# Chlumsky/msdfgen

Measured on AMD Instinct MI355X. Metric: MSDF glyphs/sec (64x64, fp32), higher is better.
Workload: dtype f64

## Files before the change

### msdfgen_amd/csrc/msdf_device.hpp

```cpp
#pragma once

#include <stdint.h>
#include <stddef.h>
#include <math.h>
#include <float.h>

#if defined(__HIPCC__)
#define MSDF_HD __host__ __device__ inline
#define MSDF_NOINLINE __attribute__((noinline))
#define MSDF_NOUNROLL _Pragma("clang loop unroll(disable)")
#define MSDF_UNROLL _Pragma("unroll")
#if defined(__HIP_DEVICE_COMPILE__)
#define MSDF_UNIFORM(x) __builtin_amdgcn_readfirstlane(x)
#else
#define MSDF_UNIFORM(x) (x)
#endif
#else
#define MSDF_HD inline
#define MSDF_NOINLINE
#define MSDF_NOUNROLL
#define MSDF_UNROLL
#define MSDF_UNIFORM(x) (x)
#endif

// ... 107 lines not shown
MSDF_HD V2 EdgeRec::EP0() const { return ld(ep0); }
MSDF_HD V2 EdgeRec::EP1() const { return ld(ep1); }

MSDF_HD V2 normalize(V2 a, bool allowZero) {
    double len = vlen(a);
    if (len != 0)
        return mk(a.x/len, a.y/len);
    return mk(0, allowZero ? 0. : 1.);
}

MSDF_HD V2 normalizeLen(V2 a, double len, bool allowZero) {
    if (len != 0)
        return mk(a.x/len, a.y/len);
    return mk(0, allowZero ? 0. : 1.);
}

MSDF_HD V2 orthonormalFalse(V2 a) {
    double len = vlen(a);
    if (len != 0)
        return mk(a.y/len, -a.x/len);
    return mk(0, -1.);
}

MSDF_HD V2 mixv(V2 a, V2 b, double w) { return (1.-w)*a+w*b; }
MSDF_HD double nonZeroSign(double n) { return n > 0 ? 1. : -1.; }
MSDF_HD double dmin(double a, double b) { return b < a ? b : a; }
MSDF_HD double dmax(double a, double b) { return a < b ? b : a; }
MSDF_HD double cmax(double a, double b) { return __builtin_fmax(a, b); }
MSDF_HD double cmin(double a, double b) { return __builtin_fmin(a, b); }
MSDF_HD double median(double a, double b, double c) { return dmax(dmin(a, b), dmin(dmax(a, b), c)); }
MSDF_HD float fmin_(float a, float b) { return b < a ? b : a; }
MSDF_HD float fmax_(float a, float b) { return a < b ? b : a; }
MSDF_HD float medianf(float a, float b, float c) { return fmax_(fmin_(a, b), fmin_(fmax_(a, b), c)); }
MSDF_HD float mixf(float a, float b, double w) { return (float) ((1.-w)*a+w*b); }

MSDF_HD double divExact(double a, double b, double y) {
    const double q = a*y;
    const double r = fma(-b, q, a);
    return fma(r, y, q);
}

MSDF_HD bool divSafe(double b) {
    const double m = fabs(b);
    if (!(m > 1e-100 && m < 1e100))
        return false;
    int e;
    const double f = frexp(m, &e);
    return f != 1-0x1p-53;
}


MSDF_HD int solveQuadratic(double x[2], double a, double b, double c) {
    if (a == 0 || fabs(b) > 1e12*fabs(a)) {
        if (b == 0) {
            if (c == 0)
                return -1;
            return 0;
        }
        x[0] = -c/b;
        return 1;
    }
    double dscr = b*b-4*a*c;
    if (dscr > 0) {
        dscr = msdfSqrt(dscr);
        x[0] = (-b+dscr)/(2*a);
        x[1] = (-b-dscr)/(2*a);
// ... 890 lines not shown
```

### msdfgen_amd/csrc/msdf_ec.hpp

```cpp
#pragma once

#include "msdf_device.hpp"

namespace msdfhip {

enum { EC_ERROR = 1, EC_PROTECTED = 2 };
enum { EC_MODE_DISABLED = 0, EC_MODE_INDISCRIMINATE = 1, EC_MODE_EDGE_PRIORITY = 2, EC_MODE_EDGE_ONLY = 3 };
enum { EC_DO_NOT_CHECK = 0, EC_CHECK_AT_EDGE = 1, EC_ALWAYS_CHECK = 2 };

#define MSDF_ARTIFACT_T_EPSILON .01
#define MSDF_PROTECTION_RADIUS_TOLERANCE 1.001

struct SdfView {
    const float *px;
    int w, h, N;
    int flip;
    MSDF_HD const float *native(int x, int y) const { return px+((size_t) y*w+x)*N; }
    MSDF_HD const float *shape(int x, int y) const { return native(x, flip ? h-1-y : y); }
};

struct EcParams {
    Xform t;
    double minDeviationRatio, minImproveRatio;
    float radiusH, radiusV, radiusD;
// ... 104 lines not shown
    l = clampi(l, sdf.w-1), r = clampi(r, sdf.w-1);
    b = clampi(b, sdf.h-1), t = clampi(t, sdf.h-1);
    const float *lb = sdf.shape(l, b), *rb = sdf.shape(r, b), *lt = sdf.shape(l, t), *rt = sdf.shape(r, t);
    for (int i = 0; i < 3; ++i)
        out[i] = mixf(mixf(lb[i], rb[i], lr), mixf(lt[i], rt[i], lr), bt);
}

template <class Query>
MSDF_HD bool evaluate(const Classifier<Query> &c, double t, float m, int flags) {
    (void) m;
    if (!c.shapeAware)
        return (flags&2) != 0;
    if (flags&1) {
        if (flags&2)
            return true;
        V2 tVector = t*c.direction;
        float oldMSD[3], newMSD[3];
        V2 sdfCoord = c.sdfCoord+tVector;
        interpolate3(oldMSD, *c.sdf, sdfCoord);
        double aWeight = (1-fabs(tVector.x))*(1-fabs(tVector.y));
        float aPSD = medianf(c.msd[0], c.msd[1], c.msd[2]);
        newMSD[0] = (float) (oldMSD[0]+aWeight*(aPSD-c.msd[0]));
        newMSD[1] = (float) (oldMSD[1]+aWeight*(aPSD-c.msd[1]));
        newMSD[2] = (float) (oldMSD[2]+aWeight*(aPSD-c.msd[2]));
        float oldPSD = medianf(oldMSD[0], oldMSD[1], oldMSD[2]);
        float newPSD = medianf(newMSD[0], newMSD[1], newMSD[2]);
        V2 q = c.shapeCoord+mk(tVector.x*c.p->texelX, tVector.y*c.p->texelY);
        float refPSD = mapDistance(c.p->t, (*c.query)(q));
        return c.p->minImproveRatio*fabsf(newPSD-refPSD) < (double) fabsf(oldPSD-refPSD);
    }
    return false;
}

MSDF_HD float interpolatedMedianLin(const float *a, const float *b, double t) {
    return medianf(mixf(a[0], b[0], t), mixf(a[1], b[1], t), mixf(a[2], b[2], t));
}

MSDF_HD float interpolatedMedianQuad(const float *a, const float *l, const float *q, double t) {
    return (float) median(t*(t*q[0]+l[0])+a[0], t*(t*q[1]+l[1])+a[1], t*(t*q[2]+l[2])+a[2]);
}

template <class Query>
MSDF_HD bool hasLinearArtifactInner(const Classifier<Query> &cl, float am, float bm, const float *a, const float *b, float dA, float dB) {
    double t = (double) dA/(dA-dB);
    if (t > MSDF_ARTIFACT_T_EPSILON && t < 1-MSDF_ARTIFACT_T_EPSILON) {
        float xm = interpolatedMedianLin(a, b, t);
        return evaluate(cl, t, xm, rangeTest(cl, 0, 1, t, am, bm, xm));
    }
    return false;
}

template <class Query>
MSDF_HD bool hasDiagonalArtifactInner(const Classifier<Query> &cl, float am, float dm, const float *a, const float *l, const float *q,
                                      float dA, float dBC, float dD, double tEx0, double tEx1) {
    double t[2];
    int solutions = solveQuadratic(t, dD-dBC+dA, dBC-dA-dA, dA);
    for (int i = 0; i < solutions; ++i) {
        if (t[i] > MSDF_ARTIFACT_T_EPSILON && t[i] < 1-MSDF_ARTIFACT_T_EPSILON) {
            float xm = interpolatedMedianQuad(a, l, q, t[i]);
            int rangeFlags = rangeTest(cl, 0, 1, t[i], am, dm, xm);
            if (tEx0 > 0 && tEx0 < 1) {
                double tEnd0 = 0, tEnd1 = 1;
                float em0 = am, em1 = dm;
                float ex = interpolatedMedianQuad(a, l, q, tEx0);
                if (tEx0 > t[i])
                    tEnd1 = tEx0, em1 = ex;
                else
                    tEnd0 = tEx0, em0 = ex;
                rangeFlags |= rangeTest(cl, tEnd0, tEnd1, t[i], em0, em1, xm);
            }
            if (tEx1 > 0 && tEx1 < 1) {
// ... 134 lines not shown
```

### msdfgen_amd/csrc/msdf_ec_fast.hpp

```cpp
#pragma once

#include "msdf_ec.hpp"

namespace msdfhip {

enum { EC_DEFER = 0x80 };

enum { EC_V_ERROR = 1,
       EC_V_CHECK = 2,
       EC_V_COND = 4,
       EC_V_HELD = 8 };
enum { EC_ORDER_EAGER = 0, EC_ORDER_LAZY = 1, EC_ORDER_LAZY_HELD = 2 };

MSDF_HD bool ecHasBasePass(const EcParams &p) { return p.distanceCheck == EC_DO_NOT_CHECK || (p.distanceCheck == EC_CHECK_AT_EDGE && p.mode != EC_MODE_EDGE_ONLY); }
MSDF_HD bool ecHasShapePass(const EcParams &p) { return p.distanceCheck == EC_ALWAYS_CHECK || p.distanceCheck == EC_CHECK_AT_EDGE; }
MSDF_HD bool ecLazyProtect(const EcParams &p) { return p.mode == EC_MODE_EDGE_PRIORITY && p.distanceCheck == EC_CHECK_AT_EDGE; }

struct FastCtx {
    double span;
    bool p1;
    bool pShape;
    bool basePass, shapePass;
    int order;
};

MSDF_HD int rangeTest2(const FastCtx &c, double at, double bt, double xt, float am, float bm, float xm) {
    const bool inversion = (am > .5f && bm > .5f && xm <= .5f) || (am < .5f && bm < .5f && xm >= .5f);
    const bool outside = medianf(am, bm, xm) != xm;
    const bool candBase = c.basePass && (inversion || (!c.p1 && outside));
    const bool candShape = c.shapePass && (inversion || (!c.pShape && outside));
    const bool candCond = c.order != EC_ORDER_EAGER && !inversion && outside;
    if (!(candBase || candShape || candCond))
        return 0;
    const double axSpan = (xt-at)*c.span, bxSpan = (bt-xt)*c.span;
    const int f = (xm >= am-axSpan && xm <= am+axSpan && xm >= bm-bxSpan && xm <= bm+bxSpan) ? 1 : 3;
    return (candBase ? f : 0)|(candShape ? f<<2 : 0)|(candCond && f == 3 ? 16 : 0);
}

MSDF_HD int judge(int flags) {
    const int cond = (flags&16) ? EC_V_COND : 0;
    if (flags&2)
        return EC_V_ERROR|cond;
    const int fs = (flags>>2)&3;
    if (fs&1)
        return ((fs&2) ? EC_V_ERROR : EC_V_CHECK)|cond;
    return cond;
}

MSDF_HD bool quadraticMayHaveRootInRange(double a, double b, double c) {
    if (a == 0 || fabs(b) > 1e12*fabs(a))
        return true;
    const double lo = .005, hi = .995;
    const double mag = fabs(a)+fabs(b)+fabs(c);
    const double eps = 1e-9*mag;
    const double flo = (a*lo+b)*lo+c, fhi = (a*hi+b)*hi+c;
    if (!(flo > eps && fhi > eps) && !(flo < -eps && fhi < -eps))
        return true;
    const double s = flo > 0 ? 1. : -1.;
    const double as = a*s, bs = b*s, cs = c*s;
    if (as <= 0)
        return false;
    if (!(-bs > 2*as*lo*(1-1e-9) && -bs < 2*as*hi*(1+1e-9)))
        return false;
    return !(4*as*cs-bs*bs > 1e-9*mag*mag);
}

MSDF_HD bool bernsteinMayHaveRoot(float dA, float dBC, float dD) {
    const float m = fmaxf(fmaxf(fabsf(dA), fabsf(dBC)), fabsf(dD));
    const float eps = 1e-5f*m;
    const float h = .5f*dBC;
    return !((dA > eps && h > eps && dD > eps) || (dA < -eps && h < -eps && dD < -eps));
}

MSDF_HD bool edgeBetweenTexelsChannelFast(const float *a, const float *b, int channel) {
    const double n = a[channel]-.5;
    const double d = a[channel]-b[channel];
    if (!((n > 0 && d > 0 && n < d) || (n < 0 && d < 0 && n > d)))
        return false;
    const double t = n/d;
    if (t > 0 && t < 1) {
        float c[3] = { mixf(a[0], b[0], t), mixf(a[1], b[1], t), mixf(a[2], b[2], t) };
        return medianf(c[0], c[1], c[2]) == c[channel];
    }
    return false;
}

MSDF_HD int edgeBetweenTexelsFast(const float *a, const float *b) {
    return 1*(int) edgeBetweenTexelsChannelFast(a, b, 0)+2*(int) edgeBetweenTexelsChannelFast(a, b, 1)+4*(int) edgeBetweenTexelsChannelFast(a, b, 2);
}

struct DiagonalRoots {
    double r0, r1;
    double ex0, ex1;
    int m, ne;
};

MSDF_HD bool diagonalRootsInRange(DiagonalRoots &d, double qa, double qb, double qc, float l0, float q0, float l1, float q1) {
    d.m = 0, d.ne = 0;
    d.r0 = d.r1 = d.ex0 = d.ex1 = 0;
    if (!quadraticMayHaveRootInRange(qa, qb, qc))
        return false;
    double t[2] = { 0, 0 };
    const int solutions = solveQuadratic(t, qa, qb, qc);
    const bool in0 = (solutions > 0)&(t[0] > MSDF_ARTIFACT_T_EPSILON)&(t[0] < 1-MSDF_ARTIFACT_T_EPSILON);
    const bool in1 = (solutions > 1)&(t[1] > MSDF_ARTIFACT_T_EPSILON)&(t[1] < 1-MSDF_ARTIFACT_T_EPSILON);
    d.m = (int) in0+(int) in1;
    if (!d.m)
        return false;
    d.r0 = in0 ? t[0] : t[1], d.r1 = t[1];
    const double tEx0 = -.5*l0/q0, tEx1 = -.5*l1/q1;
    const bool e0 = (tEx0 > 0)&(tEx0 < 1), e1 = (tEx1 > 0)&(tEx1 < 1);
    d.ne = (int) e0+(int) e1;
    d.ex0 = e0 ? tEx0 : tEx1, d.ex1 = tEx1;
    return true;
}

MSDF_HD int diagonalUnitFlags(const FastCtx &cx, float am, float dm, const float *a, const float *l, const float *q, double t, double tEx, bool extremum, float xm) {
    if (!extremum)
        return rangeTest2(cx, 0, 1, t, am, dm, xm);
    double tEnd0 = 0, tEnd1 = 1;
    float em0 = am, em1 = dm;
    const float ex = interpolatedMedianQuad(a, l, q, tEx);
    if (tEx > t)
        tEnd1 = tEx, em1 = ex;
    else
        tEnd0 = tEx, em0 = ex;
    return rangeTest2(cx, tEnd0, tEnd1, t, em0, em1, xm);
}

template <class Sink>
MSDF_HD bool diagonalRootVerdict(const FastCtx &cx, int rangeFlags, double t, int &verdict, Sink &sink) {
    const int v = judge(rangeFlags);
    verdict |= v;
    if (v&EC_V_CHECK) {
        const bool held = (verdict&EC_V_COND) != 0;
        if (held)
            verdict |= EC_V_HELD;
        if (held == (cx.order == EC_ORDER_LAZY_HELD))
            sink(t);
    }
    return (verdict&EC_V_ERROR) != 0;
}

template <class Sink>
MSDF_HD int diagonalPairFast(const FastCtx &cx, float am, float dm, const float *a, const float *l, const float *q,
                             float dA, float dBC, float dD, float l0, float q0, float l1, float q1, Sink &sink) {
    const double qa = dD-dBC+dA, qb = dBC-dA-dA, qc = dA;
    DiagonalRoots d;
    if (!diagonalRootsInRange(d, qa, qb, qc, l0, q0, l1, q1))
        return 0;
    int verdict = 0;
    MSDF_UNROLL
    for (int i = 0; i < 2; ++i) {
        if (i >= d.m)
            break;
        const double t = i ? d.r1 : d.r0;
        const float xm = interpolatedMedianQuad(a, l, q, t);
        int rangeFlags = diagonalUnitFlags(cx, am, dm, a, l, q, t, 0, false, xm);
        if (d.ne > 0)
            rangeFlags |= diagonalUnitFlags(cx, am, dm, a, l, q, t, d.ex0, true, xm);
        if (d.ne > 1)
            rangeFlags |= diagonalUnitFlags(cx, am, dm, a, l, q, t, d.ex1, true, xm);
        if (diagonalRootVerdict(cx, rangeFlags, t, verdict, sink))
            return verdict;
    }
    return verdict;
}

struct Neighbourhood {
    float v[3][3][3];
    float dev[3][3];
    unsigned cls[3][3];
    unsigned valid;
};

MSDF_HD float ecTexelDeviation(const float *t) { return fabsf(medianf(t[0], t[1], t[2])-.5f); }

enum { EC_CLS_INSIDE = 0x8000 };
MSDF_HD unsigned ecTexelClassWord(const float *t) {
    unsigned w = EC_CLS_INSIDE;
    MSDF_UNROLL
    for (int j = 0; j < 3; ++j) {
        const float d = t[j == 2 ? 0 : j+1]-t[j];
        w |= (d > 0 ? 1u<<j : 0u)|(d < 0 ? 8u<<j : 0u)|(d == 0 ? 64u<<j : 0u);
    }
    return w;
}

MSDF_HD unsigned ecValidFromWords(const Neighbourhood &nb) {
    unsigned valid = 0;
    MSDF_UNROLL
    for (int m = 0; m < 9; ++m)
        valid |= (nb.cls[m/3][m%3]&EC_CLS_INSIDE) ? 1u<<m : 0u;
    return valid;
}

MSDF_HD void loadNeighbourhood(Neighbourhood &nb, const SdfView &sdf, int x, int yn) {
    MSDF_UNROLL
    for (int dy = -1; dy <= 1; ++dy) {
        MSDF_UNROLL
        for (int dx = -1; dx <= 1; ++dx) {
            const int nx = x+dx, ny = yn+dy;
            const bool in = nx >= 0 && ny >= 0 && nx < sdf.w && ny < sdf.h;
            const float *t = sdf.native(in ? nx : x, in ? ny : yn);
            nb.v[dy+1][dx+1][0] = t[0], nb.v[dy+1][dx+1][1] = t[1], nb.v[dy+1][dx+1][2] = t[2];
            nb.dev[dy+1][dx+1] = ecTexelDeviation(t);
            nb.cls[dy+1][dx+1] = in ? ecTexelClassWord(t) : 0u;
        }
    }
    nb.valid = ecValidFromWords(nb);
}

template <class Emit>
MSDF_HD void texelProtectPairs(const Neighbourhood &nb, const EcParams &p, Emit &emit) {
    const float sdev = nb.dev[1][1];
    MSDF_UNROLL
    for (int dy = -1; dy <= 1; ++dy) {
        MSDF_UNROLL
        for (int dx = -1; dx <= 1; ++dx) {
            if (!dx && !dy)
                continue;
            if (!(nb.cls[dy+1][dx+1]&EC_CLS_INSIDE))
                continue;
            const float radius = dy == 0 ? p.radiusH : dx == 0 ? p.radiusV : p.radiusD;
            const float odev = nb.dev[dy+1][dx+1];
            const bool selfIsA = dy > 0 || (dy == 0 && dx > 0);
            const float sum = selfIsA ? sdev+odev : odev+sdev;
            if (sum < radius)
                emit((dy+1)*3+(dx+1));
        }
    }
}

MSDF_HD bool evaluateProtectPair(const float *self, const float *other, int m, bool swapRows = false) {
    const int dy = m/3-1, dx = m%3-1;
    const bool selfIsA = (swapRows ? dy < 0 : dy > 0) || (dy == 0 && dx > 0);
    const int mask = selfIsA ? edgeBetweenTexelsFast(self, other) : edgeBetweenTexelsFast(other, self);
    return extremeChannelInMask(self, medianf(self[0], self[1], self[2]), mask);
}

MSDF_HD bool protectedByEdgesNb(const Neighbourhood &nb, const EcParams &p, int flip = 0) {
    struct Items {
        unsigned char m[8];
        int n;
        MSDF_HD void operator()(int mm) { m[n++] = (unsigned char) mm; }
    } items;
    items.n = 0;
    texelProtectPairs(nb, p, items);
    for (int i = 0; i < items.n; ++i)
        if (evaluateProtectPair(nb.v[1][1], nb.v[items.m[i]/3][items.m[i]%3], items.m[i], p.shapeRows && flip))
            return true;
    return false;
}

MSDF_HD int ecNeighbourDx(int k) { return k < 4 ? (k == 0 ? -1 : k == 2 ? 1 : 0) : ((k&1) ? 1 : -1); }
MSDF_HD int ecNeighbourDy(int k) { return k < 4 ? (k == 1 ? -1 : k == 3 ? 1 : 0) : ((k&2) ? 1 : -1); }

template <class Emit>
MSDF_HD void texelCandidatePairs(const Neighbourhood &nb, Emit &emit) {
    const float *c = nb.v[1][1];
    const float cdev = nb.dev[1][1];
    const unsigned cw = nb.cls[1][1];
    MSDF_UNROLL
    for (int k = 0; k < 4; ++k) {
        const int dx = k == 0 ? -1 : k == 2 ? 1 : 0, dy = k == 1 ? -1 : k == 3 ? 1 : 0;
        const unsigned nw = nb.cls[dy+1][dx+1];
        const unsigned opposite = ((cw&(nw>>3))|((cw>>3)&nw))&7u;
        const unsigned m = cdev >= nb.dev[dy+1][dx+1] ? opposite : 0u;
        if (m) {
            if (m&1u)
                emit(k, 0);
            if (m&2u)
                emit(k, 1);
            if (m&4u)
                emit(k, 2);
        }
    }
    MSDF_UNROLL
    for (int k = 4; k < 8; ++k) {
        const int dx = (k&1) ? 1 : -1, dy = (k&2) ? 1 : -1;
        const unsigned dw = nb.cls[dy+1][dx+1];
        if (!(((dw&EC_CLS_INSIDE) != 0)&(cdev >= nb.dev[dy+1][dx+1])))
            continue;
        const float *d = nb.v[dy+1][dx+1];
        const float *b = nb.v[1][dx+1], *cc = nb.v[dy+1][1];
        const unsigned zeroAD = cw&dw;
        MSDF_UNROLL
        for (int j = 0; j < 3; ++j) {
            const int i0 = j, i1 = j == 2 ? 0 : j+1;
            const float dA = c[i1]-c[i0], dBC = b[i1]-b[i0]+cc[i1]-cc[i0], dD = d[i1]-d[i0];
            if ((zeroAD&(64u<<j)) && dBC == 0)
                continue;
            if (bernsteinMayHaveRoot(dA, dBC, dD))
                emit(k, j);
        }
    }
}

MSDF_HD float pick3(const float *v, int i) { return i == 0 ? v[0] : i == 1 ? v[1] : v[2]; }

template <class Sink>
MSDF_HD int evaluatePair(const float *c, const float *n, const float *hb, const float *vc, const EcParams &p, bool p1, int flip, int k, int j, Sink &sink,
                         int order = EC_ORDER_EAGER) {
    FastCtx cx;
    cx.basePass = ecHasBasePass(p);
    cx.shapePass = ecHasShapePass(p);
    cx.order = order;
    cx.p1 = order != EC_ORDER_EAGER || p1;
    cx.pShape = (p.distanceCheck == EC_CHECK_AT_EDGE) ? true : cx.p1;
    const int dx = ecNeighbourDx(k), dy = ecNeighbourDy(k);
    const int i0 = j, i1 = j == 2 ? 0 : j+1;
    const float cm = medianf(c[0], c[1], c[2]), nm = medianf(n[0], n[1], n[2]);
    if (k < 4) {
        if (order == EC_ORDER_LAZY_HELD)
            return 0;
        cx.span = dy == 0 ? p.hSpan : p.vSpan;
        const float dA = pick3(c, i1)-pick3(c, i0), dB = pick3(n, i1)-pick3(n, i0);
        const double t = (double) dA/(dA-dB);
        if (t > MSDF_ARTIFACT_T_EPSILON && t < 1-MSDF_ARTIFACT_T_EPSILON) {
            const float xm = interpolatedMedianLin(c, n, t);
            const int v = judge(rangeTest2(cx, 0, 1, t, cm, nm, xm));
            if (v&EC_V_CHECK)
                sink(t, dx, flip ? -dy : dy);
            return v;
        }
        return 0;
    }
    cx.span = p.dSpan;
    const float *a = c, *b = hb, *cc = vc, *d = n;
    const float abc[3] = { a[0]-b[0]-cc[0], a[1]-b[1]-cc[1], a[2]-b[2]-cc[2] };
    const float l[3] = { -a[0]-abc[0], -a[1]-abc[1], -a[2]-abc[2] };
    const float q[3] = { d[0]+abc[0], d[1]+abc[1], d[2]+abc[2] };
    const float a3[3] = { a[0], a[1], a[2] };
    struct DirSink {
        Sink &sink;
        int dx, dy;
        MSDF_HD void operator()(double t) { sink(t, dx, dy); }
    } dirSink = { sink, dx, flip ? -dy : dy };
    const float dA = pick3(a, i1)-pick3(a, i0), dBC = pick3(b, i1)-pick3(b, i0)+pick3(cc, i1)-pick3(cc, i0), dD = pick3(d, i1)-pick3(d, i0);
    return diagonalPairFast(cx, cm, nm, a3, l, q, dA, dBC, dD, pick3(l, i0), pick3(q, i0), pick3(l, i1), pick3(q, i1), dirSink);
}

template <class Sink>
MSDF_HD int texelFindFast(const Neighbourhood &nb, const EcParams &p, bool p1, int flip, Sink &sink, int order = EC_ORDER_EAGER) {
    struct Items {
        unsigned char k[24], j[24];
        int n;
        MSDF_HD void operator()(int kk, int jj) { k[n] = (unsigned char) kk, j[n] = (unsigned char) jj; ++n; }
    } items;
    items.n = 0;
    texelCandidatePairs(nb, items);
    int verdict = 0;
    for (int i = 0; i < items.n; ++i) {
        const int k = items.k[i], dx = ecNeighbourDx(k), dy = ecNeighbourDy(k);
        verdict |= evaluatePair(nb.v[1][1], nb.v[dy+1][dx+1], nb.v[1][dx+1], nb.v[dy+1][1], p, p1, flip, k, items.j[i], sink, order);
    }
    return verdict;
}

MSDF_HD bool protectedByCornerList(const int *corners, int nCorners, int x, int ys) {
    for (int i = 0; i < nCorners; ++i) {
        const int l = corners[2*i], b = corners[2*i+1];
        if ((x == l || x == l+1) && (ys == b || ys == b+1))
            return true;
    }
    return false;
}

MSDF_HD bool ecNeedsProtection(int verdict) { return ((verdict&EC_V_COND) && !(verdict&EC_V_ERROR)) || (verdict&EC_V_HELD); }

template <class Sink>
MSDF_HD int ecTexelFast(const SdfView &sdf, const EcParams &p, const int *corners, int nCorners, int x, int yn, Sink &sink, bool allowLazy = true) {
    const int ys = sdf.flip ? sdf.h-1-yn : yn;
    Neighbourhood nb;
    loadNeighbourhood(nb, sdf, x, yn);
    int st = 0, verdict;
    if (allowLazy && ecLazyProtect(p)) {
        verdict = texelFindFast(nb, p, true, sdf.flip, sink, EC_ORDER_LAZY);
        if (ecNeedsProtection(verdict)) {
            if (!(protectedByCornerList(corners, nCorners, x, ys) || protectedByEdgesNb(nb, p, sdf.flip)))
                verdict |= EC_V_ERROR;
            else if (verdict&EC_V_HELD)
                texelFindFast(nb, p, true, sdf.flip, sink, EC_ORDER_LAZY_HELD);
        }
    } else {
        if (p.mode == EC_MODE_EDGE_PRIORITY) {
            if (protectedByCornerList(corners, nCorners, x, ys) || protectedByEdgesNb(nb, p, sdf.flip))
                st |= EC_PROTECTED;
// ... 33 lines not shown
```

### msdfgen_amd/csrc/msdf_kernels.hpp

```cpp
#pragma once

#include <hip/hip_runtime.h>
#include "msdf_device.hpp"
#include "msdf_prep.hpp"
#include "msdf_ec.hpp"
#include "msdf_ec_fast.hpp"
#include "msdf_cull.hpp"
#include "msdf_scanline.hpp"
#include "msdf_shapeprep.hpp"
#include "msdf_frame.hpp"
#include "msdf_legacy.hpp"
#include "../../include/msdfgen_hip.h"

namespace msdfhip {

#ifndef MSDF_DISTANCE_WAVES_PER_SIMD
#define MSDF_DISTANCE_WAVES_PER_SIMD 4
#endif
constexpr int TILE = 8;
constexpr int WAVE = 64;
constexpr int REC_DOUBLES = sizeof(EdgeRec)/sizeof(double);

struct BatchView {
    int nGlyphs;
// ... 1013 lines not shown

#ifndef MSDF_EC_FAST_WAVES_PER_SIMD
#define MSDF_EC_FAST_WAVES_PER_SIMD 7
#endif
enum { EC_HALO = TILE+2, EC_QUEUE_CAP = WAVE*24, EC_PROTECT_QUEUE_CAP = WAVE*8 };
__host__ __device__ inline size_t ecFastLdsBytes(int maxEdges, int n) {
    return (size_t) EC_HALO*EC_HALO*n*sizeof(float)+(WAVE+4)*sizeof(int)
           +(EC_QUEUE_CAP+EC_PROTECT_QUEUE_CAP)*sizeof(unsigned short);
}

__device__ __forceinline__ bool ecTileCornerTexel(const int *list, int nCorners, int tx, int ty, int height, int flip, int lane) {
    const int lxT = lane&(TILE-1), lyT = lane>>3;
    const int xT = tx*TILE+lxT, ysT = flip ? height-1-(ty*TILE+lyT) : ty*TILE+lyT;
    const int x0 = tx*TILE, x1 = tx*TILE+TILE-1;
    const int ya = flip ? height-1-(ty*TILE+TILE-1) : ty*TILE, yb = flip ? height-1-ty*TILE : ty*TILE+TILE-1;
    bool cornerTexel = false;
    for (int base = 0; base < nCorners; base += WAVE) {
        const int k = base+lane;
        int l = 0, b = 0;
        bool near = false;
        if (k < nCorners) {
            l = list[2*k], b = list[2*k+1];
            near = l+1 >= x0 && l <= x1 && b+1 >= ya && b <= yb;
        }
        for (unsigned long long mask = __ballot(near); mask; mask &= mask-1) {
            const int src = __ffsll((long long) mask)-1;
            const int cl = __builtin_amdgcn_readlane(l, src), cb = __builtin_amdgcn_readlane(b, src);
            cornerTexel = cornerTexel || ((xT == cl || xT == cl+1) && (ysT == cb || ysT == cb+1));
        }
    }
    return cornerTexel;
}

template <int N>
__device__ __forceinline__ void ecRunProtectQueue(const float *halo, const unsigned short *protectQueue, int nProtect, int *verdictLds, int lane, bool swapRows = false) {
    for (int base = 0; base < nProtect; base += WAVE) {
        const int it = base+lane;
        if (it >= nProtect)
            continue;
        const unsigned item = protectQueue[it];
        const int s = item&63, m = item>>6;
        const int sx = s&(TILE-1), sy = s>>3;
        const float *self = halo+((sy+1)*EC_HALO+sx+1)*N, *other = halo+((sy+m/3)*EC_HALO+sx+m%3)*N;
        if (evaluateProtectPair(self, other, m, swapRows))
            atomicOr(&verdictLds[s], 0x100);
    }
}

struct EcPushProtect {
    unsigned short *queue;
    int *count;
    int lane;
    __device__ void operator()(int m) { queue[atomicAdd(count, 1)] = (unsigned short) (lane|m<<6); }
};

template <int N, int ORDER = -1, bool SIZED = false, bool SHAPE_ROWS = false>
__device__ __forceinline__ void ecFastBody(const BatchView &batch, const MsdfHipGlyph *glyphs, int width, int height, int tilesX, int tilesPerGlyph,
          const float *src, float *out, uint8_t *stencilOut, const MsdfHipConfig &cfg, const EcGlyphParams *glyphParams, EcCandidate *cands, unsigned seg,
          int maxEdges, const int *corners, const unsigned blockId, int *smemFast, const int sinkSlots = 0, const int sinkSlot = 0, const int32_t *__restrict__ dims = NULL) {
    const GlyphWork wk = decodeItem(blockId, batch.nGlyphs, tilesPerGlyph);
    if (!wk.valid)
        return;
    const int boxW = SIZED ? MSDF_UNIFORM(dims[2*wk.g]) : width, boxH = SIZED ? MSDF_UNIFORM(dims[2*wk.g+1]) : height;
    if (SIZED && ((wk.tile%tilesX)*TILE >= boxW || (wk.tile/tilesX)*TILE >= boxH))
        return;
    float *halo = reinterpret_cast<float *>(smemFast);
    int *verdictLds = reinterpret_cast<int *>(halo+EC_HALO*EC_HALO*N);
    int *itemCount = verdictLds+WAVE;
    unsigned short *queue = reinterpret_cast<unsigned short *>(itemCount+4);
    unsigned short *protectQueue = queue+EC_QUEUE_CAP;
    struct TexelClass {
        float dev;
        unsigned cls;
    };
    TexelClass *classLds = reinterpret_cast<TexelClass *>(queue+EC_QUEUE_CAP)-EC_HALO*EC_HALO;
    static_assert((EC_QUEUE_CAP*sizeof(unsigned short))%sizeof(TexelClass) == 0 && EC_QUEUE_CAP*sizeof(unsigned short) >= EC_HALO*EC_HALO*sizeof(TexelClass)
                  && 2*WAVE >= EC_HALO*EC_HALO && WAVE%EC_HALO == 4 && WAVE/EC_HALO == 6, "classLds overlays the queue's tail; the halo is staged in two rounds");
    const int lane = threadIdx.x;
    const MsdfHipGlyph gd = glyphs[wk.g];
    EcParams p;
    p.t = loadXform(gd);
    p.minDeviationRatio = cfg.min_deviation_ratio;
    p.minImproveRatio = cfg.min_improve_ratio;
    p.mode = cfg.ec_mode, p.distanceCheck = cfg.ec_distance_check, p.overlap = cfg.overlap_support, p.stageLimit = 0;
    const EcGlyphParams gp = glyphParams[wk.g];
    p.hSpan = gp.hSpan, p.vSpan = gp.vSpan, p.dSpan = gp.dSpan, p.texelX = gp.texelX, p.texelY = gp.texelY;
    p.radiusH = gp.radiusH, p.radiusV = gp.radiusV, p.radiusD = gp.radiusD;
    const int tx = wk.tile%tilesX, ty = wk.tile/tilesX;

    const bool lazy = ORDER < 0 ? ecLazyProtect(p) : ORDER != 0;
    bool cornerTexel = false;
    if (p.mode == EC_MODE_EDGE_PRIORITY && !lazy)
        cornerTexel = ecTileCornerTexel(corners+2*(size_t) gp.cornerBegin, gp.nCorners, tx, ty, boxH, gd.flip, lane);

    const ptrdiff_t rowStep = (ptrdiff_t) boxW*N;
    const ptrdiff_t origin = SIZED ? ((ptrdiff_t) wk.g*width*height+(ptrdiff_t) (ty*TILE-1)*boxW+tx*TILE-1)*N : (((ptrdiff_t) wk.g*height+ty*TILE-1)*width+tx*TILE-1)*N;
    const int hr0 = lane/EC_HALO, hc0 = lane-hr0*EC_HALO;
    const ptrdiff_t laneStep0 = hr0*rowStep+hc0*N;
    MSDF_UNROLL
    for (int round = 0; round < 2; ++round) {
        const int idx = lane+round*WAVE;
        const bool wrap = round && hc0+WAVE%EC_HALO >= EC_HALO;
        const int hc = hc0+round*(WAVE%EC_HALO)-(wrap ? EC_HALO : 0), hr = hr0+round*(WAVE/EC_HALO)+(wrap ? 1 : 0);
        const ptrdiff_t laneStep = laneStep0+round*((WAVE/EC_HALO)*rowStep+(WAVE%EC_HALO)*N)+(wrap ? rowStep-EC_HALO*N : 0);
        if (idx < EC_HALO*EC_HALO) {
            const int hx = tx*TILE+hc-1, hy = ty*TILE+hr-1;
            unsigned cls = 0;
            if (hx >= 0 && hy >= 0 && hx < boxW && hy < boxH) {
                const float *t = src+(origin+laneStep);
                float tv[N];
                for (int ch = 0; ch < N; ++ch)
                    tv[ch] = t[ch], halo[idx*N+ch] = tv[ch];
                classLds[idx].dev = ecTexelDeviation(tv);
                cls = ecTexelClassWord(tv);
            }
            classLds[idx].cls = cls;
        }
    }
    if (lane < 2)
        itemCount[lane] = 0;
    waveSync();

    const int lx = lane&(TILE-1), ly = lane>>3;
    const int x = tx*TILE+lx, yn = ty*TILE+ly;
    const bool inside = x < boxW && yn < boxH;
    int st = 0;
    const bool classify = inside;
    Neighbourhood nb;
    const int centre = (ly+1)*EC_HALO+lx+1;
    MSDF_UNROLL
    for (int dy = -1; dy <= 1; ++dy) {
        MSDF_UNROLL
        for (int dx = -1; dx <= 1; ++dx) {
            const TexelClass tc = classLds[centre+dy*EC_HALO+dx];
            nb.dev[dy+1][dx+1] = tc.dev, nb.cls[dy+1][dx+1] = tc.cls;
        }
    }
    waveSync();
    if (classify) {
        MSDF_UNROLL
        for (int dy = -1; dy <= 1; ++dy) {
            MSDF_UNROLL
            for (int dx = -1; dx <= 1; ++dx) {
                const float *t = halo+(centre+dy*EC_HALO+dx)*N;
                nb.v[dy+1][dx+1][0] = t[0], nb.v[dy+1][dx+1][1] = t[1], nb.v[dy+1][dx+1][2] = t[2];
            }
        }
        if (p.mode == EC_MODE_EDGE_PRIORITY && !lazy) {
            if (cornerTexel)
                st |= EC_PROTECTED;
            if (!(st&EC_PROTECTED)) {
                EcPushProtect pushProtect = { protectQueue, itemCount+1, lane };
                texelProtectPairs(nb, p, pushProtect);
            }
        } else if (p.mode == EC_MODE_EDGE_ONLY)
            st |= EC_PROTECTED;
        struct Push {
            unsigned short *queue;
            int *count;
            int lane;
            __device__ void operator()(int k, int j) { queue[atomicAdd(count, 1)] = (unsigned short) (lane|k<<6|j<<9); }
        } push = { queue, itemCount, lane };
        texelCandidatePairs(nb, push);
    }
    verdictLds[lane] = (st&EC_PROTECTED) ? 0x100 : 0;
    waveSync();

    if (!lazy) {
        ecRunProtectQueue<N>(halo, protectQueue, itemCount[1], verdictLds, lane, SHAPE_ROWS && gd.flip);
        waveSync();
    }

    const int nItems = itemCount[0];
    const auto runItems = [&](const int order) {
        for (int base = 0; base < nItems; base += WAVE) {
            const int it = base+lane;
            if (it >= nItems)
                continue;
            const unsigned item = queue[it];
            const int s = item&63, k = (item>>6)&7, jp = item>>9;
            const int word = verdictLds[s];
            if (order == EC_ORDER_LAZY_HELD && (word&(0x100|EC_V_HELD)) != (0x100|EC_V_HELD))
                continue;
            const int sx = s&(TILE-1), sy = s>>3;
            const int dx = ecNeighbourDx(k), dy = ecNeighbourDy(k);
            const float *c = halo+((sy+1)*EC_HALO+sx+1)*N, *n = halo+((sy+1+dy)*EC_HALO+sx+1+dx)*N;
            const float *hb = halo+((sy+1)*EC_HALO+sx+1+dx)*N, *vc = halo+((sy+1+dy)*EC_HALO+sx+1)*N;
            CandidateSink sink;
            sink.header = reinterpret_cast<unsigned *>(cands);
            sink.segment = sinkSlots > 0 ? cands+ecHeaderRecords(sinkSlots)+(size_t) sinkSlot*seg : cands+ecHeaderRecords(batch.nGlyphs)+(size_t) wk.g*seg;
            sink.seg = seg, sink.g = sinkSlots > 0 ? sinkSlot : wk.g;
            sink.texel = (unsigned) (SIZED ? (size_t) wk.g*width*height+(size_t) (ty*TILE+sy)*boxW+tx*TILE+sx : ((size_t) wk.g*height+ty*TILE+sy)*width+tx*TILE+sx);
            const int v = evaluatePair(c, n, hb, vc, p, (word&0x100) != 0, gd.flip, k, jp, sink, order);
            if (v && order != EC_ORDER_LAZY_HELD)
                atomicOr(&verdictLds[s], v);
        }
    };
    runItems(lazy ? EC_ORDER_LAZY : EC_ORDER_EAGER);
    waveSync();

    const bool need = lazy && inside && ecNeedsProtection(verdictLds[lane]);
    if (__ballot(need)) {
        __asm__ volatile("" ::: "memory");
        const EcGlyphParams gl = glyphParams[wk.g];
        EcParams pr = p;
        pr.radiusH = gl.radiusH, pr.radiusV = gl.radiusV, pr.radiusD = gl.radiusD;
        cornerTexel = ecTileCornerTexel(corners+2*(size_t) gl.cornerBegin, gl.nCorners, tx, ty, boxH, gd.flip, lane);
        if (need) {
            if (cornerTexel)
                verdictLds[lane] |= 0x100;
            else {
                Neighbourhood nd;
                MSDF_UNROLL
                for (int dy = -1; dy <= 1; ++dy) {
                    MSDF_UNROLL
                    for (int dx = -1; dx <= 1; ++dx) {
                        const int nx = x+dx, ny = yn+dy;
                        const bool in = nx >= 0 && ny >= 0 && nx < boxW && ny < boxH;
                        nd.dev[dy+1][dx+1] = ecTexelDeviation(halo+((ly+1+(in ? dy : 0))*EC_HALO+lx+1+(in ? dx : 0))*N);
                        nd.cls[dy+1][dx+1] = in ? (unsigned) EC_CLS_INSIDE : 0u;
                    }
                }
                EcPushProtect pushProtect = { protectQueue, itemCount+1, lane };
                texelProtectPairs(nd, pr, pushProtect);
            }
        }
        waveSync();
        ecRunProtectQueue<N>(halo, protectQueue, itemCount[1], verdictLds, lane);
        waveSync();
        bool revisit = false;
        if (need) {
            const int word = verdictLds[lane];
            if (!(word&0x100))
                verdictLds[lane] = word|EC_V_ERROR;
            revisit = (word&0x100) && (word&EC_V_HELD);
        }
        if (__ballot(revisit)) {
            waveSync();
            runItems(EC_ORDER_LAZY_HELD);
        }
    }

    if (!inside)
        return;
    const int verdict = verdictLds[lane];
    if ((verdict&0x100) || (ecHasBasePass(p) && p.distanceCheck == EC_CHECK_AT_EDGE))
        st |= EC_PROTECTED;
    if (verdict&EC_V_ERROR)
        st |= EC_ERROR;
    const size_t texel = SIZED ? (size_t) wk.g*width*height+(size_t) yn*boxW+x : ((size_t) wk.g*height+yn)*width+x;
    const float *in = halo+((ly+1)*EC_HALO+lx+1)*N;
    float v[N];
    for (int i = 0; i < N; ++i)
        v[i] = in[i];
    if (st&EC_ERROR) {
        const float m = medianf(v[0], v[1], v[2]);
        v[0] = m, v[1] = m, v[2] = m;
    }
    float *px = out+gd.out_offset+(ptrdiff_t) gd.row_stride*yn+(ptrdiff_t) N*x;
    for (int i = 0; i < N; ++i)
        px[i] = v[i];
    if (stencilOut)
        stencilOut[stencilIndex(texel, yn, boxW, boxH, cfg.stencil_y_down)] = (uint8_t) st;
}
template <int N, bool LAZY, bool SHAPE_ROWS = false>
__global__ void __launch_bounds__(WAVE, MSDF_EC_FAST_WAVES_PER_SIMD)
k_ec_fast(BatchView batch, const MsdfHipGlyph *glyphs, int width, int height, int tilesX, int tilesPerGlyph,
          const float *src, float *out, uint8_t *stencilOut, MsdfHipConfig cfg, const EcGlyphParams *glyphParams, EcCandidate *cands, unsigned seg,
          int maxEdges, const int *corners) {
    extern __shared__ int smemFast[];
    static_assert(!(LAZY && SHAPE_ROWS), "the lazy order's protection round pairs texels along the bitmap's rows");
    ecFastBody<N, LAZY ? 1 : 0, false, SHAPE_ROWS>(batch, glyphs, width, height, tilesX, tilesPerGlyph, src, out, stencilOut, cfg, glyphParams, cands, seg, maxEdges, corners, blockIdx.x, smemFast);
}

// ... 1048 lines not shown
```

Measured before the change: 1.891 million.

## Use hardware med3 in error correction with wave-uniform fallback and constant-folded order

Adds a hardware fmed3-based median path for the error-correction pair evaluation and protection passes. The path is chosen per wave by ballot: it is used only when all halo texel values are finite and below a magnitude bound, otherwise the original software median runs. It also constant-folds the EC mode, distance check and evaluation order for the non-sized ORDER==1 kernel, and uses direct channel indexing instead of pick3 selects. This cuts compare/select instruction count, but both variants of the sweep are instantiated, which grows code size and may raise register pressure.

```diff
diff --git a/msdfgen_amd/csrc/msdf_device.hpp b/msdfgen_amd/csrc/msdf_device.hpp
--- a/msdfgen_amd/csrc/msdf_device.hpp
+++ b/msdfgen_amd/csrc/msdf_device.hpp
@@ -163,6 +163,45 @@
 MSDF_HD float fmin_(float a, float b) { return b < a ? b : a; }
 MSDF_HD float fmax_(float a, float b) { return a < b ? b : a; }
 MSDF_HD float medianf(float a, float b, float c) { return fmax_(fmin_(a, b), fmin_(fmax_(a, b), c)); }
+MSDF_HD float med3Max(float a, float b) {
+    if (a == 0 && b == 0)
+        return (__builtin_signbit(a) && __builtin_signbit(b)) ? a : 0.f;
+    return a < b ? b : a;
+}
+MSDF_HD float med3Min(float a, float b) {
+    if (a != a)
+        return b;
+    if (b != b)
+        return a;
+    if (a == 0 && b == 0)
+        return (__builtin_signbit(a) || __builtin_signbit(b)) ? -0.f : 0.f;
+    return b < a ? b : a;
+}
+MSDF_HD float med3Model(float a, float b, float c) {
+    if (a != a || b != b || c != c)
+        return med3Min(med3Min(a, b), c);
+    const float m = med3Max(med3Max(a, b), c);
+    if (m == a)
+        return med3Max(b, c);
+    if (m == b)
+        return med3Max(a, c);
+    return med3Max(a, b);
+}
+MSDF_HD float med3f(float a, float b, float c) {
+#if defined(__HIP_DEVICE_COMPILE__)
+    return __builtin_amdgcn_fmed3f(a, b, c);
+#else
+    return med3Model(a, b, c);
+#endif
+}
+template <bool HWMED>
+MSDF_HD float medianOf(float a, float b, float c) {
+    if (HWMED)
+        return med3f(a, b, c);
+    return medianf(a, b, c);
+}
+MSDF_HD float med3Lo(float a, float b) { return __builtin_fminf(a, b); }
+MSDF_HD float med3Hi(float a, float b) { return __builtin_fmaxf(a, b); }
 MSDF_HD float mixf(float a, float b, double w) { return (float) ((1.-w)*a+w*b); }
 
 MSDF_HD double divExact(double a, double b, double y) {
diff --git a/msdfgen_amd/csrc/msdf_ec.hpp b/msdfgen_amd/csrc/msdf_ec.hpp
--- a/msdfgen_amd/csrc/msdf_ec.hpp
+++ b/msdfgen_amd/csrc/msdf_ec.hpp
@@ -160,11 +160,15 @@
     return false;
 }
 
+template <bool HWMED = false>
 MSDF_HD float interpolatedMedianLin(const float *a, const float *b, double t) {
-    return medianf(mixf(a[0], b[0], t), mixf(a[1], b[1], t), mixf(a[2], b[2], t));
-}
-
+    return medianOf<HWMED>(mixf(a[0], b[0], t), mixf(a[1], b[1], t), mixf(a[2], b[2], t));
+}
+
+template <bool HWMED = false>
 MSDF_HD float interpolatedMedianQuad(const float *a, const float *l, const float *q, double t) {
+    if (HWMED)
+        return med3f((float) (t*(t*q[0]+l[0])+a[0]), (float) (t*(t*q[1]+l[1])+a[1]), (float) (t*(t*q[2]+l[2])+a[2]));
     return (float) median(t*(t*q[0]+l[0])+a[0], t*(t*q[1]+l[1])+a[1], t*(t*q[2]+l[2])+a[2]);
 }
 
diff --git a/msdfgen_amd/csrc/msdf_ec_fast.hpp b/msdfgen_amd/csrc/msdf_ec_fast.hpp
--- a/msdfgen_amd/csrc/msdf_ec_fast.hpp
+++ b/msdfgen_amd/csrc/msdf_ec_fast.hpp
@@ -24,9 +24,11 @@
     int order;
 };
 
+template <bool HWMED = false>
 MSDF_HD int rangeTest2(const FastCtx &c, double at, double bt, double xt, float am, float bm, float xm) {
-    const bool inversion = (am > .5f && bm > .5f && xm <= .5f) || (am < .5f && bm < .5f && xm >= .5f);
-    const bool outside = medianf(am, bm, xm) != xm;
+    const bool inversion = HWMED ? (med3Lo(am, bm) > .5f && xm <= .5f) || (med3Hi(am, bm) < .5f && xm >= .5f)
+                                 : (am > .5f && bm > .5f && xm <= .5f) || (am < .5f && bm < .5f && xm >= .5f);
+    const bool outside = medianOf<HWMED>(am, bm, xm) != xm;
     const bool candBase = c.basePass && (inversion || (!c.p1 && outside));
     const bool candShape = c.shapePass && (inversion || (!c.pShape && outside));
     const bool candCond = c.order != EC_ORDER_EAGER && !inversion && outside;
@@ -72,6 +74,7 @@
     return !((dA > eps && h > eps && dD > eps) || (dA < -eps && h < -eps && dD < -eps));
 }
 
+template <bool HWMED = false>
 MSDF_HD bool edgeBetweenTexelsChannelFast(const float *a, const float *b, int channel) {
     const double n = a[channel]-.5;
     const double d = a[channel]-b[channel];
@@ -80,13 +83,14 @@
     const double t = n/d;
     if (t > 0 && t < 1) {
         float c[3] = { mixf(a[0], b[0], t), mixf(a[1], b[1], t), mixf(a[2], b[2], t) };
-        return medianf(c[0], c[1], c[2]) == c[channel];
+        return medianOf<HWMED>(c[0], c[1], c[2]) == c[channel];
     }
     return false;
 }
 
+template <bool HWMED = false>
 MSDF_HD int edgeBetweenTexelsFast(const float *a, const float *b) {
-    return 1*(int) edgeBetweenTexelsChannelFast(a, b, 0)+2*(int) edgeBetweenTexelsChannelFast(a, b, 1)+4*(int) edgeBetweenTexelsChannelFast(a, b, 2);
+    return 1*(int) edgeBetweenTexelsChannelFast<HWMED>(a, b, 0)+2*(int) edgeBetweenTexelsChannelFast<HWMED>(a, b, 1)+4*(int) edgeBetweenTexelsChannelFast<HWMED>(a, b, 2);
 }
 
 struct DiagonalRoots {
@@ -115,17 +119,18 @@
     return true;
 }
 
+template <bool HWMED = false>
 MSDF_HD int diagonalUnitFlags(const FastCtx &cx, float am, float dm, const float *a, const float *l, const float *q, double t, double tEx, bool extremum, float xm) {
     if (!extremum)
-        return rangeTest2(cx, 0, 1, t, am, dm, xm);
+        return rangeTest2<HWMED>(cx, 0, 1, t, am, dm, xm);
     double tEnd0 = 0, tEnd1 = 1;
     float em0 = am, em1 = dm;
-    const float ex = interpolatedMedianQuad(a, l, q, tEx);
+    const float ex = interpolatedMedianQuad<HWMED>(a, l, q, tEx);
     if (tEx > t)
         tEnd1 = tEx, em1 = ex;
     else
         tEnd0 = tEx, em0 = ex;
-    return rangeTest2(cx, tEnd0, tEnd1, t, em0, em1, xm);
+    return rangeTest2<HWMED>(cx, tEnd0, tEnd1, t, em0, em1, xm);
 }
 
 template <class Sink>
@@ -142,7 +147,7 @@
     return (verdict&EC_V_ERROR) != 0;
 }
 
-template <class Sink>
+template <bool HWMED = false, class Sink>
 MSDF_HD int diagonalPairFast(const FastCtx &cx, float am, float dm, const float *a, const float *l, const float *q,
                              float dA, float dBC, float dD, float l0, float q0, float l1, float q1, Sink &sink) {
     const double qa = dD-dBC+dA, qb = dBC-dA-dA, qc = dA;
@@ -155,12 +160,12 @@
         if (i >= d.m)
             break;
         const double t = i ? d.r1 : d.r0;
-        const float xm = interpolatedMedianQuad(a, l, q, t);
-        int rangeFlags = diagonalUnitFlags(cx, am, dm, a, l, q, t, 0, false, xm);
+        const float xm = interpolatedMedianQuad<HWMED>(a, l, q, t);
+        int rangeFlags = diagonalUnitFlags<HWMED>(cx, am, dm, a, l, q, t, 0, false, xm);
         if (d.ne > 0)
-            rangeFlags |= diagonalUnitFlags(cx, am, dm, a, l, q, t, d.ex0, true, xm);
+            rangeFlags |= diagonalUnitFlags<HWMED>(cx, am, dm, a, l, q, t, d.ex0, true, xm);
         if (d.ne > 1)
-            rangeFlags |= diagonalUnitFlags(cx, am, dm, a, l, q, t, d.ex1, true, xm);
+            rangeFlags |= diagonalUnitFlags<HWMED>(cx, am, dm, a, l, q, t, d.ex1, true, xm);
         if (diagonalRootVerdict(cx, rangeFlags, t, verdict, sink))
             return verdict;
     }
@@ -174,7 +179,8 @@
     unsigned valid;
 };
 
-MSDF_HD float ecTexelDeviation(const float *t) { return fabsf(medianf(t[0], t[1], t[2])-.5f); }
+template <bool HWMED = false>
+MSDF_HD float ecTexelDeviation(const float *t) { return fabsf(medianOf<HWMED>(t[0], t[1], t[2])-.5f); }
 
 enum { EC_CLS_INSIDE = 0x8000 };
 MSDF_HD unsigned ecTexelClassWord(const float *t) {
@@ -232,11 +238,12 @@
     }
 }
 
+template <bool HWMED = false>
 MSDF_HD bool evaluateProtectPair(const float *self, const float *other, int m, bool swapRows = false) {
     const int dy = m/3-1, dx = m%3-1;
     const bool selfIsA = (swapRows ? dy < 0 : dy > 0) || (dy == 0 && dx > 0);
-    const int mask = selfIsA ? edgeBetweenTexelsFast(self, other) : edgeBetweenTexelsFast(other, self);
-    return extremeChannelInMask(self, medianf(self[0], self[1], self[2]), mask);
+    const int mask = selfIsA ? edgeBetweenTexelsFast<HWMED>(self, other) : edgeBetweenTexelsFast<HWMED>(other, self);
+    return extremeChannelInMask(self, medianOf<HWMED>(self[0], self[1], self[2]), mask);
 }
 
 MSDF_HD bool protectedByEdgesNb(const Neighbourhood &nb, const EcParams &p, int flip = 0) {
@@ -298,28 +305,32 @@
 }
 
 MSDF_HD float pick3(const float *v, int i) { return i == 0 ? v[0] : i == 1 ? v[1] : v[2]; }
-
-template <class Sink>
+template <bool INDEXED>
+MSDF_HD float pickChannel(const float *v, int i) { return INDEXED ? v[i] : pick3(v, i); }
+
+template <bool HWMED = false, bool INDEXED = false, int CORDER = -1, class Sink>
 MSDF_HD int evaluatePair(const float *c, const float *n, const float *hb, const float *vc, const EcParams &p, bool p1, int flip, int k, int j, Sink &sink,
-                         int order = EC_ORDER_EAGER) {
+                         int orderArg = EC_ORDER_EAGER) {
+    const int order = CORDER >= 0 ? CORDER : orderArg;
+    constexpr bool LAZY_CT = CORDER == EC_ORDER_LAZY || CORDER == EC_ORDER_LAZY_HELD;
     FastCtx cx;
-    cx.basePass = ecHasBasePass(p);
-    cx.shapePass = ecHasShapePass(p);
+    cx.basePass = LAZY_CT || ecHasBasePass(p);
+    cx.shapePass = LAZY_CT || ecHasShapePass(p);
     cx.order = order;
     cx.p1 = order != EC_ORDER_EAGER || p1;
-    cx.pShape = (p.distanceCheck == EC_CHECK_AT_EDGE) ? true : cx.p1;
+    cx.pShape = (LAZY_CT || p.distanceCheck == EC_CHECK_AT_EDGE) ? true : cx.p1;
     const int dx = ecNeighbourDx(k), dy = ecNeighbourDy(k);
     const int i0 = j, i1 = j == 2 ? 0 : j+1;
-    const float cm = medianf(c[0], c[1], c[2]), nm = medianf(n[0], n[1], n[2]);
+    const float cm = medianOf<HWMED>(c[0], c[1], c[2]), nm = medianOf<HWMED>(n[0], n[1], n[2]);
     if (k < 4) {
         if (order == EC_ORDER_LAZY_HELD)
             return 0;
         cx.span = dy == 0 ? p.hSpan : p.vSpan;
-        const float dA = pick3(c, i1)-pick3(c, i0), dB = pick3(n, i1)-pick3(n, i0);
+        const float dA = pickChannel<INDEXED>(c, i1)-pickChannel<INDEXED>(c, i0), dB = pickChannel<INDEXED>(n, i1)-pickChannel<INDEXED>(n, i0);
         const double t = (double) dA/(dA-dB);
         if (t > MSDF_ARTIFACT_T_EPSILON && t < 1-MSDF_ARTIFACT_T_EPSILON) {
-            const float xm = interpolatedMedianLin(c, n, t);
-            const int v = judge(rangeTest2(cx, 0, 1, t, cm, nm, xm));
+            const float xm = interpolatedMedianLin<HWMED>(c, n, t);
+            const int v = judge(rangeTest2<HWMED>(cx, 0, 1, t, cm, nm, xm));
             if (v&EC_V_CHECK)
                 sink(t, dx, flip ? -dy : dy);
             return v;
@@ -337,11 +348,13 @@
         int dx, dy;
         MSDF_HD void operator()(double t) { sink(t, dx, dy); }
     } dirSink = { sink, dx, flip ? -dy : dy };
-    const float dA = pick3(a, i1)-pick3(a, i0), dBC = pick3(b, i1)-pick3(b, i0)+pick3(cc, i1)-pick3(cc, i0), dD = pick3(d, i1)-pick3(d, i0);
-    return diagonalPairFast(cx, cm, nm, a3, l, q, dA, dBC, dD, pick3(l, i0), pick3(q, i0), pick3(l, i1), pick3(q, i1), dirSink);
-}
-
-template <class Sink>
+    const float dA = pickChannel<INDEXED>(a, i1)-pickChannel<INDEXED>(a, i0);
+    const float dBC = pickChannel<INDEXED>(b, i1)-pickChannel<INDEXED>(b, i0)+pickChannel<INDEXED>(cc, i1)-pickChannel<INDEXED>(cc, i0);
+    const float dD = pickChannel<INDEXED>(d, i1)-pickChannel<INDEXED>(d, i0);
+    return diagonalPairFast<HWMED>(cx, cm, nm, a3, l, q, dA, dBC, dD, pick3(l, i0), pick3(q, i0), pick3(l, i1), pick3(q, i1), dirSink);
+}
+
+template <bool HWMED = false, class Sink>
 MSDF_HD int texelFindFast(const Neighbourhood &nb, const EcParams &p, bool p1, int flip, Sink &sink, int order = EC_ORDER_EAGER) {
     struct Items {
         unsigned char k[24], j[24];
@@ -353,7 +366,7 @@
     int verdict = 0;
     for (int i = 0; i < items.n; ++i) {
         const int k = items.k[i], dx = ecNeighbourDx(k), dy = ecNeighbourDy(k);
-        verdict |= evaluatePair(nb.v[1][1], nb.v[dy+1][dx+1], nb.v[1][dx+1], nb.v[dy+1][1], p, p1, flip, k, items.j[i], sink, order);
+        verdict |= evaluatePair<HWMED>(nb.v[1][1], nb.v[dy+1][dx+1], nb.v[1][dx+1], nb.v[dy+1][1], p, p1, flip, k, items.j[i], sink, order);
     }
     return verdict;
 }
diff --git a/msdfgen_amd/csrc/msdf_kernels.hpp b/msdfgen_amd/csrc/msdf_kernels.hpp
--- a/msdfgen_amd/csrc/msdf_kernels.hpp
+++ b/msdfgen_amd/csrc/msdf_kernels.hpp
@@ -1069,7 +1069,7 @@
     return cornerTexel;
 }
 
-template <int N>
+template <int N, bool HWMED = false>
 __device__ __forceinline__ void ecRunProtectQueue(const float *halo, const unsigned short *protectQueue, int nProtect, int *verdictLds, int lane, bool swapRows = false) {
     for (int base = 0; base < nProtect; base += WAVE) {
         const int it = base+lane;
@@ -1079,10 +1079,15 @@
         const int s = item&63, m = item>>6;
         const int sx = s&(TILE-1), sy = s>>3;
         const float *self = halo+((sy+1)*EC_HALO+sx+1)*N, *other = halo+((sy+m/3)*EC_HALO+sx+m%3)*N;
-        if (evaluateProtectPair(self, other, m, swapRows))
+        if (evaluateProtectPair<HWMED>(self, other, m, swapRows))
             atomicOr(&verdictLds[s], 0x100);
     }
 }
+
+template <class T, T V>
+struct EcConstant {
+    static constexpr T value = V;
+};
 
 struct EcPushProtect {
     unsigned short *queue;
@@ -1119,7 +1124,9 @@
     p.t = loadXform(gd);
     p.minDeviationRatio = cfg.min_deviation_ratio;
     p.minImproveRatio = cfg.min_improve_ratio;
-    p.mode = cfg.ec_mode, p.distanceCheck = cfg.ec_distance_check, p.overlap = cfg.overlap_support, p.stageLimit = 0;
+    constexpr bool FOLD = ORDER == 1 && !SIZED;
+    p.mode = FOLD ? (int) EC_MODE_EDGE_PRIORITY : cfg.ec_mode, p.distanceCheck = FOLD ? (int) EC_CHECK_AT_EDGE : cfg.ec_distance_check;
+    p.overlap = cfg.overlap_support, p.stageLimit = 0;
     const EcGlyphParams gp = glyphParams[wk.g];
     p.hSpan = gp.hSpan, p.vSpan = gp.vSpan, p.dSpan = gp.dSpan, p.texelX = gp.texelX, p.texelY = gp.texelY;
     p.radiusH = gp.radiusH, p.radiusV = gp.radiusV, p.radiusD = gp.radiusD;
@@ -1134,6 +1141,10 @@
     const ptrdiff_t origin = SIZED ? ((ptrdiff_t) wk.g*width*height+(ptrdiff_t) (ty*TILE-1)*boxW+tx*TILE-1)*N : (((ptrdiff_t) wk.g*height+ty*TILE-1)*width+tx*TILE-1)*N;
     const int hr0 = lane/EC_HALO, hc0 = lane-hr0*EC_HALO;
     const ptrdiff_t laneStep0 = hr0*rowStep+hc0*N;
+    constexpr bool VOTE = ORDER >= 0 && !SIZED && !SHAPE_ROWS;
+    constexpr bool INDEXED = VOTE;
+    constexpr float EC_MED3_BOUND = 0x1p100f;
+    bool objection = false;
     MSDF_UNROLL
     for (int round = 0; round < 2; ++round) {
         const int idx = lane+round*WAVE;
@@ -1148,6 +1159,8 @@
                 float tv[N];
                 for (int ch = 0; ch < N; ++ch)
                     tv[ch] = t[ch], halo[idx*N+ch] = tv[ch];
+                if (VOTE)
+                    objection = objection || !(fabsf(tv[0]) < EC_MED3_BOUND && fabsf(tv[1]) < EC_MED3_BOUND && fabsf(tv[2]) < EC_MED3_BOUND);
                 classLds[idx].dev = ecTexelDeviation(tv);
                 cls = ecTexelClassWord(tv);
             }
@@ -1203,13 +1216,18 @@
     verdictLds[lane] = (st&EC_PROTECTED) ? 0x100 : 0;
     waveSync();
 
+    const bool hwMedian = VOTE && __ballot(objection) == 0;
+    const auto sweep = [&](auto hwmedTag) {
+    constexpr bool HWMED = decltype(hwmedTag)::value;
     if (!lazy) {
-        ecRunProtectQueue<N>(halo, protectQueue, itemCount[1], verdictLds, lane, SHAPE_ROWS && gd.flip);
+        ecRunProtectQueue<N, HWMED>(halo, protectQueue, itemCount[1], verdictLds, lane, SHAPE_ROWS && gd.flip);
         waveSync();
     }
 
     const int nItems = itemCount[0];
-    const auto runItems = [&](const int order) {
+    const auto runItems = [&](auto orderTag, const int orderArg) {
+        constexpr int CORDER = decltype(orderTag)::value;
+        const int order = CORDER >= 0 ? CORDER : orderArg;
         for (int base = 0; base < nItems; base += WAVE) {
             const int it = base+lane;
             if (it >= nItems)
@@ -1228,12 +1246,17 @@
             sink.segment = sinkSlots > 0 ? cands+ecHeaderRecords(sinkSlots)+(size_t) sinkSlot*seg : cands+ecHeaderRecords(batch.nGlyphs)+(size_t) wk.g*seg;
             sink.seg = seg, sink.g = sinkSlots > 0 ? sinkSlot : wk.g;
             sink.texel = (unsigned) (SIZED ? (size_t) wk.g*width*height+(size_t) (ty*TILE+sy)*boxW+tx*TILE+sx : ((size_t) wk.g*height+ty*TILE+sy)*width+tx*TILE+sx);
-            const int v = evaluatePair(c, n, hb, vc, p, (word&0x100) != 0, gd.flip, k, jp, sink, order);
+            const int v = evaluatePair<HWMED, INDEXED, (FOLD || CORDER == EC_ORDER_EAGER) ? CORDER : -1>(c, n, hb, vc, p, (word&0x100) != 0, gd.flip, k, jp, sink, order);
             if (v && order != EC_ORDER_LAZY_HELD)
                 atomicOr(&verdictLds[s], v);
         }
     };
-    runItems(lazy ? EC_ORDER_LAZY : EC_ORDER_EAGER);
+    if constexpr (ORDER < 0)
+        runItems(EcConstant<int, -1>(), lazy ? EC_ORDER_LAZY : EC_ORDER_EAGER);
+    else if constexpr (ORDER == 1)
+        runItems(EcConstant<int, EC_ORDER_LAZY>(), EC_ORDER_LAZY);
+    else
+        runItems(EcConstant<int, EC_ORDER_EAGER>(), EC_ORDER_EAGER);
     waveSync();
 
     const bool need = lazy && inside && ecNeedsProtection(verdictLds[lane]);
@@ -1254,7 +1277,7 @@
                     for (int dx = -1; dx <= 1; ++dx) {
                         const int nx = x+dx, ny = yn+dy;
                         const bool in = nx >= 0 && ny >= 0 && nx < boxW && ny < boxH;
-                        nd.dev[dy+1][dx+1] = ecTexelDeviation(halo+((ly+1+(in ? dy : 0))*EC_HALO+lx+1+(in ? dx : 0))*N);
+                        nd.dev[dy+1][dx+1] = ecTexelDeviation<HWMED>(halo+((ly+1+(in ? dy : 0))*EC_HALO+lx+1+(in ? dx : 0))*N);
                         nd.cls[dy+1][dx+1] = in ? (unsigned) EC_CLS_INSIDE : 0u;
                     }
                 }
@@ -1263,7 +1286,7 @@
             }
         }
         waveSync();
-        ecRunProtectQueue<N>(halo, protectQueue, itemCount[1], verdictLds, lane);
+        ecRunProtectQueue<N, HWMED>(halo, protectQueue, itemCount[1], verdictLds, lane);
         waveSync();
         bool revisit = false;
         if (need) {
@@ -1274,9 +1297,17 @@
         }
         if (__ballot(revisit)) {
             waveSync();
-            runItems(EC_ORDER_LAZY_HELD);
-        }
-    }
+            if constexpr (ORDER < 0)
+                runItems(EcConstant<int, -1>(), EC_ORDER_LAZY_HELD);
+            else
+                runItems(EcConstant<int, EC_ORDER_LAZY_HELD>(), EC_ORDER_LAZY_HELD);
+        }
+    }
+    };
+    if (hwMedian)
+        sweep(EcConstant<bool, true>());
+    else
+        sweep(EcConstant<bool, false>());
 
     if (!inside)
         return;
```

New measurement: 1.934 million (median of 6 runs). 1.02x the previous value.
